# amazon-science/instruct-video-to-video

Hardware: AMD Instinct MI355X
Metric: denoised video-frames/sec (16f@256x384, 50 DDIM steps) (higher is better)
Workload: dtype fp16; 1 GPU; C2: 1 clip/step = VAE-encode + 50 DDIM steps (3-way CFG, text 7.5 / video 1.5) + VAE-decode, 16 frames @ 256x384, random-init full-width UNet+VAE; 5 independent clips in flight per GPU (stacked into every UNet launch, B = 3 x clips); frames=16, height=256, width=384, ddim_steps=50, clips_per_gpu=5, parallelism=clip-parallel x1, one all_gather, hip_graph=True, cfg_branch_streams=False, concurrent_clips=5, clip_mode=stacked, driver_mode=False, full=False

## Files before the change

### instruct-video-to-video_amd/csrc/winograd.hip

```cpp
#include "common.h"

namespace {

template <bool UP> __device__ __forceinline__ int lds_px(int sp) { return UP ? sp : sp ^ ((sp >> 1) & 1); }

template <bool NORM, bool UP>
__global__ __launch_bounds__(256) void wino_input_kernel(const half_t* __restrict__ x, const half_t* __restrict__ x2, const float* __restrict__ ab,
                                                         half_t* __restrict__ V, int64_t ldx, int64_t ldx2, int C1, int C, int NB, int H, int W,
                                                         int ipb, int images_per_sample, int silu, int64_t group_rows, int band_tr) {
    extern __shared__ __attribute__((aligned(16))) char smem[];
    const int tid = threadIdx.x, chunk = tid & 7, item0 = tid >> 3;
    const int nb0 = (int)blockIdx.x * ipb, c0 = (int)blockIdx.y * 64;
    const int trows = UP ? H : (H + 1) >> 1;
    const int tr0 = (int)blockIdx.z * band_tr, tr1 = min(tr0 + band_tr, trows);
    const bool whole = band_tr >= trows;
    const int row0 = whole ? 0 : (UP ? tr0 - 1 : 2 * tr0 - 1);
    const int nrows = whole ? H : (UP ? (tr1 - tr0) + 2 : 2 * (tr1 - tr0) + 2);
    const int HW = H * W, SW = nrows * W;
    const int SWs = UP ? SW : (SW + 1) & ~1;
    const bool second = x2 != nullptr && c0 >= C1;
    const half_t* src = second ? x2 + (c0 - C1) + chunk * 8 : x + c0 + chunk * 8;
    const int64_t ld = second ? ldx2 : ldx;
    const int nimg = min(ipb, NB - nb0);
    for (int it = item0; it < nimg * SW; it += 32) {
        const int img = it / SW, sp = it - img * SW;
        const int iy = row0 + sp / W;
        if ((unsigned)iy >= (unsigned)H) continue;
        half8 v = *(const half8*)(src + ((int64_t)(nb0 + img) * HW + sp + row0 * W) * ld);
        if (NORM) {
            const float* p = ab + ((int64_t)((nb0 + img) / images_per_sample) * C + c0 + chunk * 8) * 2;
            const float4 p0 = *(const float4*)p, p1 = *(const float4*)(p + 4), p2 = *(const float4*)(p + 8), p3 = *(const float4*)(p + 12);
            const float sc[8] = {p0.x, p0.z, p1.x, p1.z, p2.x, p2.z, p3.x, p3.z}, sh[8] = {p0.y, p0.w, p1.y, p1.w, p2.y, p2.w, p3.y, p3.w};
#pragma unroll
            for (int e = 0; e < 8; ++e) {
                float f = fmaf((float)v[e], sc[e], sh[e]);
                if (silu) f = silu_f(f);
                v[e] = (half_t)f;
            }
        }
        *(half8*)(smem + ((int64_t)img * SWs + lds_px<UP>(sp)) * 128 + chunk * 16) = v;
    }
    __syncthreads();
    if constexpr (UP) {
        const int bt = (tr1 - tr0) * W;
        for (int it = item0; it < nimg * bt; it += 32) {
            const int img = it / bt, tb_ = it - img * bt;
            const int y = tr0 + tb_ / W, xx = tb_ - (tb_ / W) * W;
            const int t = y * W + xx;
            const char* base = smem + (int64_t)img * SWs * 128 + chunk * 16;
            float hz[3][3][8];
#pragma unroll
            for (int r = 0; r < 3; ++r) {
                const int iy = y - 1 + r;
                float d[3][8];
#pragma unroll
                for (int c = 0; c < 3; ++c) {
                    const int ix = xx - 1 + c;
                    const bool ok = (unsigned)iy < (unsigned)H && (unsigned)ix < (unsigned)W;
                    half8 v = {0, 0, 0, 0, 0, 0, 0, 0};
                    if (ok) v = *(const half8*)(base + lds_px<UP>((iy - row0) * W + ix) * 128);
#pragma unroll
                    for (int e = 0; e < 8; ++e) d[c][e] = (float)v[e];
                }
#pragma unroll
                for (int e = 0; e < 8; ++e) {
                    hz[r][0][e] = d[0][e] - d[1][e];
                    hz[r][1][e] = 2.f * d[1][e];
                    hz[r][2][e] = d[1][e] - d[2][e];
                }
            }
            const int64_t trow = (int64_t)(nb0 + img) * HW + t;
            half_t* dst = V + trow * C + c0 + chunk * 8;
#pragma unroll
            for (int j = 0; j < 3; ++j) {
                half8 o[3];
#pragma unroll
                for (int e = 0; e < 8; ++e) {
                    o[0][e] = (half_t)(hz[0][j][e] - hz[1][j][e]);
                    o[1][e] = (half_t)(2.f * hz[1][j][e]);
                    o[2][e] = (half_t)(hz[1][j][e] - hz[2][j][e]);
                }
#pragma unroll
                for (int i = 0; i < 3; ++i) *(half8*)(dst + (int64_t)(i * 3 + j) * group_rows * C) = o[i];
            }
        }
        return;
    }
    const int th = (H + 1) >> 1, tw = (W + 1) >> 1, ntile = th * tw;
    const int bt = (tr1 - tr0) * tw;
    for (int it = item0; it < nimg * bt; it += 32) {
        const int img = it / bt, tb_ = it - img * bt;
        const int ty = tr0 + tb_ / tw, tx = tb_ - (tb_ / tw) * tw;
        const int t = ty * tw + tx;
        const char* base = smem + (int64_t)img * SWs * 128 + chunk * 16;
        float hz[4][4][8];
#pragma unroll
        for (int r = 0; r < 4; ++r) {
            const int iy = 2 * ty - 1 + r;
            float d[4][8];
#pragma unroll
            for (int c = 0; c < 4; ++c) {
                const int ix = 2 * tx - 1 + c;
                const bool ok = (unsigned)iy < (unsigned)H && (unsigned)ix < (unsigned)W;
                half8 v = {0, 0, 0, 0, 0, 0, 0, 0};
                if (ok) v = *(const half8*)(base + lds_px<UP>((iy - row0) * W + ix) * 128);
#pragma unroll
                for (int e = 0; e < 8; ++e) d[c][e] = (float)v[e];
            }
#pragma unroll
            for (int e = 0; e < 8; ++e) {
                hz[r][0][e] = d[0][e] - d[2][e];
                hz[r][1][e] = d[1][e] + d[2][e];
                hz[r][2][e] = d[2][e] - d[1][e];
                hz[r][3][e] = d[1][e] - d[3][e];
            }
        }
        const int64_t trow = (int64_t)(nb0 + img) * ntile + t;
        half_t* dst = V + trow * C + c0 + chunk * 8;
#pragma unroll
        for (int j = 0; j < 4; ++j) {
            half8 o[4];
#pragma unroll
            for (int e = 0; e < 8; ++e) {
                o[0][e] = (half_t)(hz[0][j][e] - hz[2][j][e]);
                o[1][e] = (half_t)(hz[1][j][e] + hz[2][j][e]);
                o[2][e] = (half_t)(hz[2][j][e] - hz[1][j][e]);
                o[3][e] = (half_t)(hz[1][j][e] - hz[3][j][e]);
            }
#pragma unroll
            for (int i = 0; i < 4; ++i) *(half8*)(dst + (int64_t)(i * 4 + j) * group_rows * C) = o[i];
        }
    }
}

template <bool RES, bool RB, bool UP>
__global__ __launch_bounds__(256) void wino_output_kernel(const half_t* __restrict__ Mo, const float* __restrict__ bias, const float* __restrict__ row_bias,
                                                          const half_t* __restrict__ res, half_t* __restrict__ y, int64_t group_rows, int64_t ntiles_total,
                                                          int Cout, int H, int W, int64_t ld_rb, int rows_per_group, int64_t ldr, int64_t ldy) {
    const int c8 = Cout >> 3;
    const int64_t idx = (int64_t)blockIdx.x * 256 + threadIdx.x;
    const int64_t tile = idx / c8;
    if (tile >= ntiles_total) return;
    const int ch = (int)(idx - tile * c8) * 8;
    const int th = UP ? H : (H + 1) >> 1, tw = UP ? W : (W + 1) >> 1, ntile = th * tw;
    const int OW = UP ? 2 * W : W, OH = UP ? 2 * H : H;
    const int nb = (int)(tile / ntile), t = (int)(tile - (int64_t)nb * ntile);
    const int ty = t / tw, tx = t - ty * tw;
    const half_t* src = Mo + tile * Cout + ch;
    float s[2][4][8];
    if constexpr (UP) {
#pragma unroll
        for (int j = 0; j < 3; ++j) {
            half8 m[3];
#pragma unroll
            for (int i = 0; i < 3; ++i) m[i] = *(const half8*)(src + (int64_t)(i * 3 + j) * group_rows * Cout);
            const int jj = j == 2 ? 3 : j;
#pragma unroll
            for (int e = 0; e < 8; ++e) {
                s[0][jj][e] = (float)m[0][e] + (float)m[1][e];
                s[1][jj][e] = (float)m[1][e] - (float)m[2][e];
            }
        }
#pragma unroll
        for (int e = 0; e < 8; ++e) s[0][2][e] = s[1][2][e] = 0.f;
    } else {
#pragma unroll
        for (int j = 0; j < 4; ++j) {
            half8 m[4];
#pragma unroll
            for (int i = 0; i < 4; ++i) m[i] = *(const half8*)(src + (int64_t)(i * 4 + j) * group_rows * Cout);
#pragma unroll
            for (int e = 0; e < 8; ++e) {
                s[0][j][e] = (float)m[0][e] + (float)m[1][e] + (float)m[2][e];
                s[1][j][e] = (float)m[1][e] - (float)m[2][e] - (float)m[3][e];
            }
        }
    }
    float b[8];
    {
        const float4 b0 = bias ? *(const float4*)(bias + ch) : make_float4(0.f, 0.f, 0.f, 0.f), b1 = bias ? *(const float4*)(bias + ch + 4) : make_float4(0.f, 0.f, 0.f, 0.f);
        b[0] = b0.x; b[1] = b0.y; b[2] = b0.z; b[3] = b0.w; b[4] = b1.x; b[5] = b1.y; b[6] = b1.z; b[7] = b1.w;
    }
    const int64_t m00 = ((int64_t)nb * OH + 2 * ty) * OW + 2 * tx;
    if (RB) {
        const float* rb = row_bias + (m00 / rows_per_group) * ld_rb + ch;
        const float4 r0 = *(const float4*)rb, r1 = *(const float4*)(rb + 4);
        b[0] += r0.x; b[1] += r0.y; b[2] += r0.z; b[3] += r0.w; b[4] += r1.x; b[5] += r1.y; b[6] += r1.z; b[7] += r1.w;
    }
#pragma unroll
    for (int i = 0; i < 2; ++i)
#pragma unroll
        for (int jj = 0; jj < 2; ++jj) {
            if (!UP && (2 * ty + i >= OH || 2 * tx + jj >= OW)) continue;
            const int64_t m = m00 + (int64_t)i * OW + jj;
            float v[8];
#pragma unroll
            for (int e = 0; e < 8; ++e)
                v[e] = (jj == 0 ? s[i][0][e] + s[i][1][e] + s[i][2][e] : s[i][1][e] - s[i][2][e] - s[i][3][e]) + b[e];
            if (RES) {
                const half8 r = *(const half8*)(res + m * ldr + ch);
#pragma unroll
                for (int e = 0; e < 8; ++e) v[e] += (float)r[e];
            }
            half8 o;
#pragma unroll
            for (int e = 0; e < 8; ++e) o[e] = (half_t)v[e];
            *(half8*)(y + m * ldy + ch) = o;
        }
}

}

extern "C" int insv2v_winograd_input(const insv2v_winograd_in_desc* dp, insv2v_stream_t stream) {
    if (!dp) return INSV2V_EINVAL;
    const insv2v_winograd_in_desc& d = *dp;
    if (!d.x || !d.v || d.NB <= 0 || d.H <= 0 || d.W <= 0 || d.C <= 0) return INSV2V_EINVAL;
    if ((d.C % 64) || (d.x2 && (d.C1 <= 0 || d.C1 >= d.C || (d.C1 % 64)))) return INSV2V_EUNSUPPORTED;
    if ((d.ldx & 7) || ((uintptr_t)d.x & 15) || ((uintptr_t)d.v & 15) || (d.x2 && ((d.ldx2 & 7) || ((uintptr_t)d.x2 & 15)))) return INSV2V_EINVAL;
    if (d.gn_ab && (d.gn_images_per_sample <= 0 || ((uintptr_t)d.gn_ab & 15))) return INSV2V_EINVAL;
    const int HW = d.H * d.W, ntile = d.upsample ? HW : ((d.H + 1) / 2) * ((d.W + 1) / 2);
    const int HWs = d.upsample ? HW : (HW + 1) & ~1;
    const int64_t tiles = (int64_t)d.NB * ntile;
    if (d.v_group_rows < tiles) return INSV2V_EINVAL;
    const int trows = d.upsample ? d.H : (d.H + 1) / 2;
    int band_tr = trows, ipb = 1;
    if (HWs * 128 <= 64 * 1024) {
        ipb = 32 / ntile;
        if (ipb < 1) ipb = 1;
        while (ipb > 1 && ipb * HWs * 128 > 64 * 1024) --ipb;
    } else {
        const int max_rows = 64 * 1024 / (d.W * 128);
        band_tr = d.upsample ? max_rows - 2 : (max_rows - 2) / 2;
        if (band_tr < 1) return INSV2V_EUNSUPPORTED;
    }
    const int nbands = (trows + band_tr - 1) / band_tr;
    const int srows = nbands == 1 ? d.H : (d.upsample ? band_tr + 2 : 2 * band_tr + 2);
    const dim3 grid((unsigned)((d.NB + ipb - 1) / ipb), (unsigned)(d.C / 64), (unsigned)nbands);
    const int slots = srows * d.W;
    const size_t lds = (size_t)ipb * (d.upsample ? slots : (slots + 1) & ~1) * 128;
#define WINO_IN(NORM, UP)                                                                                                                             \
    hipLaunchKernelGGL((wino_input_kernel<NORM, UP>), grid, dim3(256), lds, as_stream(stream), (const half_t*)d.x, (const half_t*)d.x2, d.gn_ab, (half_t*)d.v, \
                       d.ldx, d.ldx2, d.x2 ? d.C1 : d.C, d.C, d.NB, d.H, d.W, ipb, d.gn_ab ? d.gn_images_per_sample : 1, d.gn_ab ? d.gn_silu : 0, d.v_group_rows, band_tr)
    if (d.gn_ab) { if (d.upsample) WINO_IN(true, true); else WINO_IN(true, false); }
    else { if (d.upsample) WINO_IN(false, true); else WINO_IN(false, false); }
#undef WINO_IN
    return launch_status();
}

extern "C" int insv2v_winograd_output(const insv2v_winograd_out_desc* dp, insv2v_stream_t stream) {
    if (!dp) return INSV2V_EINVAL;
    const insv2v_winograd_out_desc& d = *dp;
    if (!d.m || !d.y || d.NB <= 0 || d.H <= 0 || d.W <= 0 || d.Cout <= 0) return INSV2V_EINVAL;
    if (d.Cout & 7) return INSV2V_EUNSUPPORTED;
    if ((d.ldy & 7) || ((uintptr_t)d.m & 15) || ((uintptr_t)d.y & 15) || (d.residual && ((d.ldr & 7) || ((uintptr_t)d.residual & 15)))) return INSV2V_EINVAL;
    if ((d.bias && ((uintptr_t)d.bias & 15)) || (d.row_bias && (((uintptr_t)d.row_bias & 15) || (d.ld_rb & 3) || d.rows_per_group <= 0 || d.rows_per_group % (d.H * d.W * (d.upsample ? 4 : 1)))))
        return INSV2V_EINVAL;
    const int64_t tiles = d.upsample ? (int64_t)d.NB * d.H * d.W : (int64_t)d.NB * ((d.H + 1) / 2) * ((d.W + 1) / 2);
    if (d.m_group_rows < tiles) return INSV2V_EINVAL;
    const int64_t n = tiles * (d.Cout / 8);
    const dim3 grid((unsigned)((n + 255) / 256));
#define WINO_OUT(RES, RB, UP)                                                                                                                        \
    hipLaunchKernelGGL((wino_output_kernel<RES, RB, UP>), grid, dim3(256), 0, as_stream(stream), (const half_t*)d.m, d.bias, d.row_bias, (const half_t*)d.residual, \
                       (half_t*)d.y, d.m_group_rows, tiles, d.Cout, d.H, d.W, d.ld_rb, d.rows_per_group, d.ldr, d.ldy)
    if (d.upsample) {
        if (d.residual) { if (d.row_bias) WINO_OUT(true, true, true); else WINO_OUT(true, false, true); }
        else { if (d.row_bias) WINO_OUT(false, true, true); else WINO_OUT(false, false, true); }
    } else {
        if (d.residual) { if (d.row_bias) WINO_OUT(true, true, false); else WINO_OUT(true, false, false); }
        else { if (d.row_bias) WINO_OUT(false, true, false); else WINO_OUT(false, false, false); }
    }
#undef WINO_OUT
    return launch_status();
}
```

Measured before the change: 16.60 frames/s.

## Restructure Winograd input transform as streaming row-sliding window kernel

Replaces the whole-image or band staging of the input tile into large dynamic LDS with a streaming scheme. Each thread owns a 2-pixel column strip and a channel slice, slides a register window down the rows of a fixed band, and exchanges halo columns with its neighbours through a small double-buffered shared array. Output stores become nontemporal. This removes the large LDS footprint, which limited occupancy, and prefetches the next row while the current one is transformed. In exchange it adds per-row barriers, re-reads halo rows at band edges, and adds a one_device check to both entry points.

```diff
diff --git a/instruct-video-to-video_amd/csrc/winograd.hip b/instruct-video-to-video_amd/csrc/winograd.hip
--- a/instruct-video-to-video_amd/csrc/winograd.hip
+++ b/instruct-video-to-video_amd/csrc/winograd.hip
@@ -2,134 +2,166 @@
 
 namespace {
 
-template <bool UP> __device__ __forceinline__ int lds_px(int sp) { return UP ? sp : sp ^ ((sp >> 1) & 1); }
+constexpr int WINO_E = 8;
+constexpr int WINO_SLICE = 256;
+constexpr int WINO_ITEMS = 8;
+constexpr int WINO_CHUNKS = WINO_SLICE / WINO_E, WINO_THREADS = WINO_ITEMS * WINO_CHUNKS;
+constexpr int WINO_BAND = 8;
+constexpr int WINO_BAND_UP = 16;
+
+__device__ __forceinline__ void store_v(half_t* p, const float (&f)[WINO_E]) {
+    half8 o;
+#pragma unroll
+    for (int e = 0; e < WINO_E; ++e) o[e] = (half_t)f[e];
+    __builtin_nontemporal_store(o, (half8*)p);
+}
 
 template <bool NORM, bool UP>
-__global__ __launch_bounds__(256) void wino_input_kernel(const half_t* __restrict__ x, const half_t* __restrict__ x2, const float* __restrict__ ab,
+__global__ __launch_bounds__(WINO_THREADS) void wino_input_kernel(const half_t* __restrict__ x, const half_t* __restrict__ x2, const float* __restrict__ ab,
                                                          half_t* __restrict__ V, int64_t ldx, int64_t ldx2, int C1, int C, int NB, int H, int W,
-                                                         int ipb, int images_per_sample, int silu, int64_t group_rows, int band_tr) {
-    extern __shared__ __attribute__((aligned(16))) char smem[];
-    const int tid = threadIdx.x, chunk = tid & 7, item0 = tid >> 3;
-    const int nb0 = (int)blockIdx.x * ipb, c0 = (int)blockIdx.y * 64;
-    const int trows = UP ? H : (H + 1) >> 1;
-    const int tr0 = (int)blockIdx.z * band_tr, tr1 = min(tr0 + band_tr, trows);
-    const bool whole = band_tr >= trows;
-    const int row0 = whole ? 0 : (UP ? tr0 - 1 : 2 * tr0 - 1);
-    const int nrows = whole ? H : (UP ? (tr1 - tr0) + 2 : 2 * (tr1 - tr0) + 2);
-    const int HW = H * W, SW = nrows * W;
-    const int SWs = UP ? SW : (SW + 1) & ~1;
-    const bool second = x2 != nullptr && c0 >= C1;
-    const half_t* src = second ? x2 + (c0 - C1) + chunk * 8 : x + c0 + chunk * 8;
+                                                         int images_per_sample, int silu, int64_t group_rows, int nstrips) {
+    constexpr int R = UP ? 1 : 2;
+    constexpr int WR = UP ? 3 : 4;
+    constexpr int NPRE = UP ? 2 : 1;
+    constexpr int BAND = UP ? WINO_BAND_UP : WINO_BAND;
+    __shared__ half8 sm[2][R][2][WINO_THREADS];
+    const int tid = threadIdx.x, chunk = tid % WINO_CHUNKS, ci = tid / WINO_CHUNKS;
+    const int strip = (int)blockIdx.x % nstrips, band = (int)blockIdx.x / nstrips;
+    const int trows = UP ? H : (H + 1) >> 1, ncol = (W + 1) >> 1;
+    const int tr0 = band * BAND, tr1 = min(tr0 + BAND, trows);
+    const int item = strip * WINO_ITEMS + ci;
+    const int nb = item / ncol, px0 = 2 * (item - nb * ncol);
+    const int c = (int)blockIdx.y * WINO_SLICE + chunk * WINO_E;
+    const bool act = c < C && nb < NB;
+    const bool second = x2 != nullptr && c >= C1;
     const int64_t ld = second ? ldx2 : ldx;
-    const int nimg = min(ipb, NB - nb0);
-    for (int it = item0; it < nimg * SW; it += 32) {
-        const int img = it / SW, sp = it - img * SW;
-        const int iy = row0 + sp / W;
-        if ((unsigned)iy >= (unsigned)H) continue;
-        half8 v = *(const half8*)(src + ((int64_t)(nb0 + img) * HW + sp + row0 * W) * ld);
-        if (NORM) {
-            const float* p = ab + ((int64_t)((nb0 + img) / images_per_sample) * C + c0 + chunk * 8) * 2;
-            const float4 p0 = *(const float4*)p, p1 = *(const float4*)(p + 4), p2 = *(const float4*)(p + 8), p3 = *(const float4*)(p + 12);
-            const float sc[8] = {p0.x, p0.z, p1.x, p1.z, p2.x, p2.z, p3.x, p3.z}, sh[8] = {p0.y, p0.w, p1.y, p1.w, p2.y, p2.w, p3.y, p3.w};
-#pragma unroll
-            for (int e = 0; e < 8; ++e) {
-                float f = fmaf((float)v[e], sc[e], sh[e]);
-                if (silu) f = silu_f(f);
-                v[e] = (half_t)f;
-            }
-        }
-        *(half8*)(smem + ((int64_t)img * SWs + lds_px<UP>(sp)) * 128 + chunk * 16) = v;
-    }
-    __syncthreads();
-    if constexpr (UP) {
-        const int bt = (tr1 - tr0) * W;
-        for (int it = item0; it < nimg * bt; it += 32) {
-            const int img = it / bt, tb_ = it - img * bt;
-            const int y = tr0 + tb_ / W, xx = tb_ - (tb_ / W) * W;
-            const int t = y * W + xx;
-            const char* base = smem + (int64_t)img * SWs * 128 + chunk * 16;
-            float hz[3][3][8];
-#pragma unroll
-            for (int r = 0; r < 3; ++r) {
-                const int iy = y - 1 + r;
-                float d[3][8];
-#pragma unroll
-                for (int c = 0; c < 3; ++c) {
-                    const int ix = xx - 1 + c;
-                    const bool ok = (unsigned)iy < (unsigned)H && (unsigned)ix < (unsigned)W;
-                    half8 v = {0, 0, 0, 0, 0, 0, 0, 0};
-                    if (ok) v = *(const half8*)(base + lds_px<UP>((iy - row0) * W + ix) * 128);
-#pragma unroll
-                    for (int e = 0; e < 8; ++e) d[c][e] = (float)v[e];
-                }
-#pragma unroll
-                for (int e = 0; e < 8; ++e) {
-                    hz[r][0][e] = d[0][e] - d[1][e];
-                    hz[r][1][e] = 2.f * d[1][e];
-                    hz[r][2][e] = d[1][e] - d[2][e];
-                }
-            }
-            const int64_t trow = (int64_t)(nb0 + img) * HW + t;
-            half_t* dst = V + trow * C + c0 + chunk * 8;
-#pragma unroll
-            for (int j = 0; j < 3; ++j) {
-                half8 o[3];
-#pragma unroll
-                for (int e = 0; e < 8; ++e) {
-                    o[0][e] = (half_t)(hz[0][j][e] - hz[1][j][e]);
-                    o[1][e] = (half_t)(2.f * hz[1][j][e]);
-                    o[2][e] = (half_t)(hz[1][j][e] - hz[2][j][e]);
-                }
-#pragma unroll
-                for (int i = 0; i < 3; ++i) *(half8*)(dst + (int64_t)(i * 3 + j) * group_rows * C) = o[i];
-            }
-        }
-        return;
-    }
-    const int th = (H + 1) >> 1, tw = (W + 1) >> 1, ntile = th * tw;
-    const int bt = (tr1 - tr0) * tw;
-    for (int it = item0; it < nimg * bt; it += 32) {
-        const int img = it / bt, tb_ = it - img * bt;
-        const int ty = tr0 + tb_ / tw, tx = tb_ - (tb_ / tw) * tw;
-        const int t = ty * tw + tx;
-        const char* base = smem + (int64_t)img * SWs * 128 + chunk * 16;
-        float hz[4][4][8];
-#pragma unroll
-        for (int r = 0; r < 4; ++r) {
-            const int iy = 2 * ty - 1 + r;
-            float d[4][8];
-#pragma unroll
-            for (int c = 0; c < 4; ++c) {
-                const int ix = 2 * tx - 1 + c;
-                const bool ok = (unsigned)iy < (unsigned)H && (unsigned)ix < (unsigned)W;
-                half8 v = {0, 0, 0, 0, 0, 0, 0, 0};
-                if (ok) v = *(const half8*)(base + lds_px<UP>((iy - row0) * W + ix) * 128);
-#pragma unroll
-                for (int e = 0; e < 8; ++e) d[c][e] = (float)v[e];
-            }
-#pragma unroll
-            for (int e = 0; e < 8; ++e) {
-                hz[r][0][e] = d[0][e] - d[2][e];
-                hz[r][1][e] = d[1][e] + d[2][e];
-                hz[r][2][e] = d[2][e] - d[1][e];
-                hz[r][3][e] = d[1][e] - d[3][e];
-            }
-        }
-        const int64_t trow = (int64_t)(nb0 + img) * ntile + t;
-        half_t* dst = V + trow * C + c0 + chunk * 8;
-#pragma unroll
-        for (int j = 0; j < 4; ++j) {
-            half8 o[4];
-#pragma unroll
-            for (int e = 0; e < 8; ++e) {
-                o[0][e] = (half_t)(hz[0][j][e] - hz[2][j][e]);
-                o[1][e] = (half_t)(hz[1][j][e] + hz[2][j][e]);
-                o[2][e] = (half_t)(hz[2][j][e] - hz[1][j][e]);
-                o[3][e] = (half_t)(hz[1][j][e] - hz[3][j][e]);
-            }
-#pragma unroll
-            for (int i = 0; i < 4; ++i) *(half8*)(dst + (int64_t)(i * 4 + j) * group_rows * C) = o[i];
-        }
+    const half_t* src = (second ? x2 + (c - C1) : x + c) + (int64_t)nb * H * W * ld;
+    const int hcol = ci == 0 ? px0 - 1 : (ci == WINO_ITEMS - 1 ? px0 + 2 : -1);
+    float sc[WINO_E], sh[WINO_E];
+    if (NORM && act) {
+        const float* p = ab + ((int64_t)(nb / images_per_sample) * C + c) * 2;
+#pragma unroll
+        for (int e = 0; e < WINO_E; e += 2) {
+            const float4 t = *(const float4*)(p + 2 * e);
+            sc[e] = t.x; sh[e] = t.y; sc[e + 1] = t.z; sh[e + 1] = t.w;
+        }
+    }
+    half8 zero;
+#pragma unroll
+    for (int e = 0; e < WINO_E; ++e) zero[e] = (half_t)0.f;
+    auto inside = [&](int s, int r, int cc) {
+        const int iy = UP ? s + 1 : 2 * s + 1 + r, ix = cc < 2 ? px0 + cc : hcol;
+        return act && (unsigned)iy < (unsigned)H && (unsigned)ix < (unsigned)W;
+    };
+    auto load_step = [&](int s, half8 (&raw)[R][3]) {
+#pragma unroll
+        for (int r = 0; r < R; ++r)
+#pragma unroll
+            for (int cc = 0; cc < 3; ++cc) {
+                const int iy = UP ? s + 1 : 2 * s + 1 + r, ix = cc < 2 ? px0 + cc : hcol;
+                raw[r][cc] = inside(s, r, cc) ? *(const half8*)(src + ((int64_t)iy * W + ix) * ld) : zero;
+            }
+    };
+    half8 win[WR][4];
+#pragma unroll
+    for (int r = 0; r < WR; ++r)
+#pragma unroll
+        for (int cc = 0; cc < 4; ++cc) win[r][cc] = zero;
+    half8 raw[R][3];
+    const int s0 = tr0 - NPRE;
+    load_step(s0, raw);
+    for (int s = s0; s < tr1; ++s) {
+        const int buf = (s - s0) & 1;
+        half8 hv[R];
+#pragma unroll
+        for (int r = 0; r < R; ++r)
+#pragma unroll
+            for (int cc = 0; cc < 3; ++cc) {
+                half8 v = raw[r][cc];
+                if (NORM && inside(s, r, cc)) {
+#pragma unroll
+                    for (int e = 0; e < WINO_E; ++e) {
+                        float f = fmaf((float)v[e], sc[e], sh[e]);
+                        if (silu) f = silu_f(f);
+                        v[e] = (half_t)f;
+                    }
+                }
+                if (cc < 2) {
+                    win[WR - R + r][1 + cc] = v;
+                    sm[buf][r][cc][tid] = v;
+                } else {
+                    hv[r] = v;
+                }
+            }
+        if (s + 1 < tr1) load_step(s + 1, raw);
+        __syncthreads();
+#pragma unroll
+        for (int r = 0; r < R; ++r) {
+            const half8 l = sm[buf][r][1][ci == 0 ? tid : tid - WINO_CHUNKS], rr = sm[buf][r][0][ci == WINO_ITEMS - 1 ? tid : tid + WINO_CHUNKS];
+            win[WR - R + r][0] = ci == 0 ? hv[r] : (px0 > 0 ? l : zero);
+            win[WR - R + r][3] = ci == WINO_ITEMS - 1 ? hv[r] : (px0 + 2 < W ? rr : zero);
+        }
+        if (s >= tr0 && act) {
+            if constexpr (UP) {
+#pragma unroll
+                for (int tb = 0; tb < 2; ++tb) {
+                    if (px0 + tb >= W) continue;
+                    float hz[3][3][WINO_E];
+#pragma unroll
+                    for (int r = 0; r < 3; ++r)
+#pragma unroll
+                        for (int e = 0; e < WINO_E; ++e) {
+                            const float d0 = (float)win[r][tb][e], d1 = (float)win[r][tb + 1][e], d2 = (float)win[r][tb + 2][e];
+                            hz[r][0][e] = d0 - d1;
+                            hz[r][1][e] = 2.f * d1;
+                            hz[r][2][e] = d1 - d2;
+                        }
+                    half_t* dst = V + ((int64_t)nb * H * W + (int64_t)s * W + px0 + tb) * C + c;
+#pragma unroll
+                    for (int j = 0; j < 3; ++j) {
+                        float o[3][WINO_E];
+#pragma unroll
+                        for (int e = 0; e < WINO_E; ++e) {
+                            o[0][e] = hz[0][j][e] - hz[1][j][e];
+                            o[1][e] = 2.f * hz[1][j][e];
+                            o[2][e] = hz[1][j][e] - hz[2][j][e];
+                        }
+#pragma unroll
+                        for (int i = 0; i < 3; ++i) store_v(dst + (int64_t)(i * 3 + j) * group_rows * C, o[i]);
+                    }
+                }
+            } else if (px0 < W) {
+                float hz[4][4][WINO_E];
+#pragma unroll
+                for (int r = 0; r < 4; ++r)
+#pragma unroll
+                    for (int e = 0; e < WINO_E; ++e) {
+                        const float d0 = (float)win[r][0][e], d1 = (float)win[r][1][e], d2 = (float)win[r][2][e], d3 = (float)win[r][3][e];
+                        hz[r][0][e] = d0 - d2;
+                        hz[r][1][e] = d1 + d2;
+                        hz[r][2][e] = d2 - d1;
+                        hz[r][3][e] = d1 - d3;
+                    }
+                half_t* dst = V + ((int64_t)nb * trows * ncol + (int64_t)s * ncol + (px0 >> 1)) * C + c;
+#pragma unroll
+                for (int j = 0; j < 4; ++j) {
+                    float o[4][WINO_E];
+#pragma unroll
+                    for (int e = 0; e < WINO_E; ++e) {
+                        o[0][e] = hz[0][j][e] - hz[2][j][e];
+                        o[1][e] = hz[1][j][e] + hz[2][j][e];
+                        o[2][e] = hz[2][j][e] - hz[1][j][e];
+                        o[3][e] = hz[1][j][e] - hz[3][j][e];
+                    }
+#pragma unroll
+                    for (int i = 0; i < 4; ++i) store_v(dst + (int64_t)(i * 4 + j) * group_rows * C, o[i]);
+                }
+            }
+        }
+#pragma unroll
+        for (int r = 0; r + R < WR; ++r)
+#pragma unroll
+            for (int cc = 0; cc < 4; ++cc) win[r][cc] = win[r + R][cc];
     }
 }
 
@@ -212,35 +244,27 @@
 }
 
 extern "C" int insv2v_winograd_input(const insv2v_winograd_in_desc* dp, insv2v_stream_t stream) {
-    if (!dp) return INSV2V_EINVAL;
+    if (!one_device() || !dp) return INSV2V_EINVAL;
     const insv2v_winograd_in_desc& d = *dp;
     if (!d.x || !d.v || d.NB <= 0 || d.H <= 0 || d.W <= 0 || d.C <= 0) return INSV2V_EINVAL;
     if ((d.C % 64) || (d.x2 && (d.C1 <= 0 || d.C1 >= d.C || (d.C1 % 64)))) return INSV2V_EUNSUPPORTED;
     if ((d.ldx & 7) || ((uintptr_t)d.x & 15) || ((uintptr_t)d.v & 15) || (d.x2 && ((d.ldx2 & 7) || ((uintptr_t)d.x2 & 15)))) return INSV2V_EINVAL;
     if (d.gn_ab && (d.gn_images_per_sample <= 0 || ((uintptr_t)d.gn_ab & 15))) return INSV2V_EINVAL;
     const int HW = d.H * d.W, ntile = d.upsample ? HW : ((d.H + 1) / 2) * ((d.W + 1) / 2);
-    const int HWs = d.upsample ? HW : (HW + 1) & ~1;
     const int64_t tiles = (int64_t)d.NB * ntile;
     if (d.v_group_rows < tiles) return INSV2V_EINVAL;
-    const int trows = d.upsample ? d.H : (d.H + 1) / 2;
-    int band_tr = trows, ipb = 1;
-    if (HWs * 128 <= 64 * 1024) {
-        ipb = 32 / ntile;
-        if (ipb < 1) ipb = 1;
-        while (ipb > 1 && ipb * HWs * 128 > 64 * 1024) --ipb;
-    } else {
+    if (((d.upsample ? HW : (HW + 1) & ~1)) * 128 > 64 * 1024) {
         const int max_rows = 64 * 1024 / (d.W * 128);
-        band_tr = d.upsample ? max_rows - 2 : (max_rows - 2) / 2;
-        if (band_tr < 1) return INSV2V_EUNSUPPORTED;
-    }
-    const int nbands = (trows + band_tr - 1) / band_tr;
-    const int srows = nbands == 1 ? d.H : (d.upsample ? band_tr + 2 : 2 * band_tr + 2);
-    const dim3 grid((unsigned)((d.NB + ipb - 1) / ipb), (unsigned)(d.C / 64), (unsigned)nbands);
-    const int slots = srows * d.W;
-    const size_t lds = (size_t)ipb * (d.upsample ? slots : (slots + 1) & ~1) * 128;
+        if ((d.upsample ? max_rows - 2 : (max_rows - 2) / 2) < 1) return INSV2V_EUNSUPPORTED;
+    }
+    const int trows = d.upsample ? d.H : (d.H + 1) / 2, ncol = (d.W + 1) / 2;
+    const int band_tr = d.upsample ? WINO_BAND_UP : WINO_BAND;
+    const int64_t nstrips = ((int64_t)d.NB * ncol + WINO_ITEMS - 1) / WINO_ITEMS, nbands = (trows + band_tr - 1) / band_tr;
+    if (nstrips * nbands > 0x7fffffff) return INSV2V_EUNSUPPORTED;
+    const dim3 grid((unsigned)(nstrips * nbands), (unsigned)((d.C + WINO_SLICE - 1) / WINO_SLICE));
 #define WINO_IN(NORM, UP)                                                                                                                             \
-    hipLaunchKernelGGL((wino_input_kernel<NORM, UP>), grid, dim3(256), lds, as_stream(stream), (const half_t*)d.x, (const half_t*)d.x2, d.gn_ab, (half_t*)d.v, \
-                       d.ldx, d.ldx2, d.x2 ? d.C1 : d.C, d.C, d.NB, d.H, d.W, ipb, d.gn_ab ? d.gn_images_per_sample : 1, d.gn_ab ? d.gn_silu : 0, d.v_group_rows, band_tr)
+    hipLaunchKernelGGL((wino_input_kernel<NORM, UP>), grid, dim3(WINO_THREADS), 0, as_stream(stream), (const half_t*)d.x, (const half_t*)d.x2, d.gn_ab, (half_t*)d.v, \
+                       d.ldx, d.ldx2, d.x2 ? d.C1 : d.C, d.C, d.NB, d.H, d.W, d.gn_ab ? d.gn_images_per_sample : 1, d.gn_ab ? d.gn_silu : 0, d.v_group_rows, (int)nstrips)
     if (d.gn_ab) { if (d.upsample) WINO_IN(true, true); else WINO_IN(true, false); }
     else { if (d.upsample) WINO_IN(false, true); else WINO_IN(false, false); }
 #undef WINO_IN
@@ -248,7 +272,7 @@
 }
 
 extern "C" int insv2v_winograd_output(const insv2v_winograd_out_desc* dp, insv2v_stream_t stream) {
-    if (!dp) return INSV2V_EINVAL;
+    if (!one_device() || !dp) return INSV2V_EINVAL;
     const insv2v_winograd_out_desc& d = *dp;
     if (!d.m || !d.y || d.NB <= 0 || d.H <= 0 || d.W <= 0 || d.Cout <= 0) return INSV2V_EINVAL;
     if (d.Cout & 7) return INSV2V_EUNSUPPORTED;
```

Result: no change. 16.63 frames/s, median of 6 (+0.2%).
